# lucian-ilie/SAGE2

Hardware: AMD Instinct MI355X
Metric: overlaps/sec + edge-set bit-identity vs OpenMP ref, 150 bp reads k=40 (higher is better)
Workload: dtype u64

## Files before the change

### sage2_amd/csrc/kernels_index.inc

```


__device__ __forceinline__ void entry_key(const u64* __restrict__ reads, int S, int h, u64 id, int t, u64& hi, u64& lo) {
    const u64* w = reads + id * S;
    int L = (int)(w[S - 1] & slot_len_mask(S));
    u64 phi, plo;
    if (t == 0 || t == 3) key_at(w, S, 0, h, phi, plo); else key_at(w, S, L - h, h, phi, plo);
    if (t >= 2) rc_key(phi, plo, h, hi, lo); else { hi = phi; lo = plo; }
}

__device__ __forceinline__ u64 quad_word(const ulonglong2& v, int q) {
    const u64 a = __shfl(v.x, q >> 1, 4), b = __shfl(v.y, q >> 1, 4);
    return (q & 1) ? b : a;
}
__device__ __forceinline__ void quad_key_at(const ulonglong2& v, int j, int h, u64& hi, u64& lo) {
    const int q = (2 * j) >> 6, r = (2 * j) & 63;
    const u64 w0 = quad_word(v, q);
    u64 w1 = quad_word(v, q + 1 < 8 ? q + 1 : q); w1 = q + 1 < 8 ? w1 : 0ull;
    const u64 a = (w0 << r) | ((w1 >> 1) >> (63 - r));
    if (h <= 32) { hi = 0; lo = a >> (64 - 2 * h); return; }
    u64 w2 = quad_word(v, q + 2 < 8 ? q + 2 : q); w2 = q + 2 < 8 ? w2 : 0ull;
    const u64 b = (w1 << r) | ((w2 >> 1) >> (63 - r));
    const int d = 2 * h - 64;
    hi = a >> (64 - d); lo = d == 64 ? b : ((a << d) | (b >> (64 - d)));
}
// ... 37 lines not shown
__global__ __launch_bounds__(PT_THREADS) void k_ix_tuples(const u64* __restrict__ reads, const u32* __restrict__ posOf, int byPos, u32 N, int S, int h, u64 seed, u32 Th, int wantMI, int shift0, u32 mask0, int doHist,
                                                         u32* T, u32* cnt, u32 ntiles) {
    __shared__ u32 hst[PT_NB_MAX];
    if (doHist) { for (u32 x = threadIdx.x; x <= mask0; x += PT_THREADS) hst[x] = 0; __syncthreads(); }
    if (S == 8) ix_quad_tile<false>(reads, posOf, byPos, N, h, seed, Th, wantMI, shift0, mask0, doHist, T, hst, nullptr);
    else {
#pragma unroll 1
    for (int j = 0; j < PT_TILE / 4 / PT_THREADS; j++) {
        const u32 id0 = blockIdx.x * (PT_TILE / 4) + j * PT_THREADS + threadIdx.x;
        if (id0 >= N) continue;
        const u64 id = (u64)id0 + 1;
        const u64 pos = posOf[id]; const u64 ent4 = pos * 4;
        const u64* w = reads + (byPos ? pos : id) * S;
        const int L = (int)(w[S - 1] & slot_len_mask(S));
        u64 khi[4], klo[4];
        key_at(w, S, 0, h, khi[0], klo[0]); key_at(w, S, L - h, h, khi[1], klo[1]);
        rc_key(khi[1], klo[1], h, khi[2], klo[2]); rc_key(khi[0], klo[0], h, khi[3], klo[3]);
        u32 kk[4], mm[4]; u64 pp[4];
#pragma unroll
        for (int t = 0; t < 4; t++) {
            const u64 hv = hash_key(khi[t], klo[t], h, seed);
            kk[t] = __umulhi((u32)(hv >> 32), Th);
            pp[t] = ((u64)tag_of(hv) << 32) | (u64)(u32)(ent4 + (u64)t);
            mm[t] = 0;
            if (wantMI) { u32 k0, k1, k2, k3; key_left_align(khi[t], klo[t], h, k0, k1, k2, k3); mm[t] = minim_hash(key_min_hash(k0, k1, k2, k3, h), (u32)seed); }
            if (doHist) atomicAdd(&hst[pt_digit(kk[t], shift0, mask0)], 1u);
        }
        if (wantMI) {
#pragma unroll
            for (int t = 0; t < 4; t++) ((uint4*)T)[4 * (u64)id0 + t] = make_uint4(kk[t], mm[t], (u32)pp[t], (u32)(pp[t] >> 32));
        } else {
            u32* o = T + 12 * (u64)id0;
#pragma unroll
            for (int t = 0; t < 4; t++) { o[3 * t] = kk[t]; o[3 * t + 1] = (u32)pp[t]; o[3 * t + 2] = (u32)(pp[t] >> 32); }
        }
    }
    }
    if (doHist) { __syncthreads(); for (u32 x = threadIdx.x; x <= mask0; x += PT_THREADS) cnt[(u64)x * ntiles + blockIdx.x] = hst[x]; }
}
__global__ __launch_bounds__(PT_THREADS) void k_ix_tuples_loc(const u64* __restrict__ reads, const u32* __restrict__ posOf, u32 N, int h, u64 seed, u32 Th, int wantMI, int shift0, u32 mask0, int doHist,
                                                             u32* T, u32* cnt, u32 ntiles, u64* loc) {
    __shared__ u32 hst[PT_NB_MAX];
    if (doHist) { for (u32 x = threadIdx.x; x <= mask0; x += PT_THREADS) hst[x] = 0; __syncthreads(); }
    if (blockIdx.x == 0 && threadIdx.x < 4) ((ulonglong2*)loc)[(u64)posOf[0] * 4 + threadIdx.x] = ((const ulonglong2*)reads)[threadIdx.x];
    ix_quad_tile<true>(reads, posOf, 0, N, h, seed, Th, wantMI, shift0, mask0, doHist, T, hst, loc);
    if (doHist) { __syncthreads(); for (u32 x = threadIdx.x; x <= mask0; x += PT_THREADS) cnt[(u64)x * ntiles + blockIdx.x] = hst[x]; }
}

__global__ void k_debug_table(const u64* __restrict__ slots, u64 T, u64* out) {
    for (u64 idx = (u64)blockIdx.x * blockDim.x + threadIdx.x; idx < T; idx += (u64)gridDim.x * blockDim.x) {
        u64 s = slots[idx]; if (s == 0) continue;
        u32 c7 = (u32)(s >> SLOT_CNT_SHIFT) & 127u;
        atomicAdd(&out[0], 1ull);
        if (c7 == 1) atomicAdd(&out[1], 1ull);
        if (c7 == 0) atomicAdd(&out[2], 1ull);
        if ((s >> SLOT_TAG_SHIFT) == 0) atomicAdd(&out[3], 1ull);
        if (c7 >= 2 && c7 < 127) atomicAdd(&out[4], (u64)c7);
    }
}
__global__ void k_debug_keys(const u64* __restrict__ reads, u64 N, int S, int h, u64* out) {
    u64 e = (u64)blockIdx.x * blockDim.x + threadIdx.x;
    if (e >= 4 * N) return;
    u64 hi, lo; entry_key(reads, S, h, (e >> 2) + 1, (int)(e & 3), hi, lo);
    out[2 * e] = hi; out[2 * e + 1] = lo;
}
template <int NWAVES> __device__ __forceinline__ u32 block_excl_scan(u32 v, u32* sh, u32& total);

constexpr int IXW_CNT_BITS_DEFAULT = 20, IXW_CNT_BITS_WIDE = 30;
__device__ u32 g_fp_mask = 0xFFFFFu;
constexpr int IXW_T = 256;
constexpr int IXW_R = 3072 / IXW_T;
constexpr int IXW_CSR_CAP = 3072;
constexpr u32 GT_INVALID = 0x80000000u;
struct IxWinArgs {
    const u32* T; int W;
    const u32* winOff; u32 nW;
    u64* slots; u32* csr; u64* counters; u64* big; u32 big_cap;
    const u32* idOf;
    u32* G;
    u32 cntBits;
    u64* wh; u64 wh_cap;
};
constexpr int IXW_WAVES = 1;
__global__ __launch_bounds__(IXW_T, IXW_WAVES) void k_ix_window(IxWinArgs A) {
    __shared__ u64 tbl[IX_W];
    __shared__ u32 csrL[IXW_CSR_CAP];
    __shared__ unsigned short csrT[IXW_CSR_CAP];
    __shared__ u32 sh[IXW_T / 64]; __shared__ u64 shWh;
    const u32 tid = threadIdx.x;
    const bool hasM = A.G != nullptr;
    auto tuple = [&](u64 i, u32& k, u64& p, u32& m) {
        if (A.W == 4) { const uint4 v = ((const uint4*)A.T)[i]; k = v.x; m = v.y; p = ((u64)v.w << 32) | v.z; }
        else { const u32* q = A.T + 3 * i; k = q[0]; m = 0; p = ((u64)q[2] << 32) | q[1]; }
    };
    const int IXW_FP_SHIFT = (int)A.cntBits; const u64 IXW_CNT = (1ull << A.cntBits) - 1ull, IXW_FP_MASK = (1ull << (40 - A.cntBits)) - 1ull;
    const u32 fpMask = g_fp_mask & (u32)IXW_FP_MASK;
    u64 accCsr = 0, accOcc = 0;
    for (u32 w = blockIdx.x; w < A.nW; w += gridDim.x) {
        for (u32 x = tid; x < (u32)IX_W; x += IXW_T) tbl[x] = 0ull;
        __syncthreads();
        const u32 b = A.winOff[w], e = A.winOff[w + 1];
        u64 whBase = 0;
        if (e - b > (u32)IXW_R * (u32)IXW_T) {
            if (tid == 0) { const u64 need = (u64)(e - b) - (u64)IXW_R * (u64)IXW_T; u64 at = atomicAdd((unsigned long long*)&A.counters[9], (unsigned long long)need);
                            if (at + need > A.wh_cap) { atomicAdd(&A.counters[8], 1ull << 40); at = ~0ull; } shWh = at; }
            __syncthreads();
            whBase = shWh;
            __syncthreads();
            if (whBase == ~0ull) continue;
        }
        auto insert = [&](u32 k, u64 p, u32 m, u32& info, u32& rank) {
            const u64 tag = p >> 32; const u64 fp = (u64)((m ^ (m >> 20)) & fpMask);
            u32 idx = (k & (u32)(IX_WP - 1)) * 2u; bool files = false; u32 rk = 0; u32 steps = 0;
            for (;;) {
                u64 s = tbl[idx];
                if (s == 0) {
                    s = atomicCAS((unsigned long long*)&tbl[idx], 0ull, (unsigned long long)((tag << SLOT_TAG_SHIFT) | (fp << IXW_FP_SHIFT) | 1ull));
                    if (s == 0) { files = true; break; }
                }
                if ((s >> SLOT_TAG_SHIFT) == tag) {
                    rk = (u32)(atomicAdd((unsigned long long*)&tbl[idx], 1ull) & IXW_CNT);
                    if (rk >= (u32)IXW_CNT - 8u) atomicAdd(&A.counters[8], 1ull << 20);
                    files = ((s >> IXW_FP_SHIFT) & IXW_FP_MASK) != fp;
                    break;
                }
                idx = (idx + 1u) & (u32)(IX_W - 1);
                if (++steps > (u32)IX_W) { atomicAdd(&A.counters[8], 1ull); idx = ~0u; break; }
            }
            info = idx == ~0u ? ~0u : (idx | (files ? 0x80000000u : 0u)); rank = rk;
        };
        u64 cp[IXW_R]; u32 cm[IXW_R], ci[IXW_R], cr[IXW_R]; u32 ck[IXW_R];
#pragma unroll
        for (int r = 0; r < IXW_R; r++) {
            const u32 i = b + (u32)r * (u32)IXW_T + tid; const bool v = i < e;
            ck[r] = 0; cp[r] = 0; cm[r] = 0; if (v) tuple(i, ck[r], cp[r], cm[r]);
        }
#pragma unroll
        for (int r = 0; r < IXW_R; r++) {
            ci[r] = ~0u; cr[r] = 0;
            if (b + (u32)r * (u32)IXW_T + tid < e) insert(ck[r], cp[r], cm[r], ci[r], cr[r]);
        }
        for (u64 i = (u64)b + (u64)IXW_R * (u64)IXW_T + tid; i < e; i += IXW_T) {
            u32 info, rank; u32 tk, tm; u64 tp; tuple(i, tk, tp, tm); insert(tk, tp, tm, info, rank);
            A.wh[whBase + (i - b - (u64)IXW_R * (u64)IXW_T)] = (u64)info | ((u64)rank << 32);
        }
        __syncthreads();
        u32 c[IX_W / IXW_T]; u32 need = 0, occ = 0;
#pragma unroll
        for (int x = 0; x < IX_W / IXW_T; x++) { c[x] = (u32)(tbl[x * IXW_T + tid] & IXW_CNT); need += c[x] >= 2 ? c[x] : 0u; occ += c[x] != 0; }
        u32 total; const u32 excl = block_excl_scan<IXW_T / 64>(need, sh, total);
        u32 occTotal; block_excl_scan<IXW_T / 64>(occ, sh, occTotal);
        accCsr += total; accOcc += occTotal;
        const u64 csrBase = b;
        const bool staged = total <= (u32)IXW_CSR_CAP && (e - b) <= 65535u;
        {
            u64 start = csrBase + excl;
#pragma unroll
            for (int x = 0; x < IX_W / IXW_T; x++) {
                if (c[x] == 0) continue;
                const u32 idx = x * IXW_T + tid; const u64 tagbits = tbl[idx] & (~0ull << SLOT_TAG_SHIFT);
                if (c[x] == 1) tbl[idx] = tagbits | (1ull << SLOT_CNT_SHIFT);
                else {
                    const u32 c7 = c[x] >= HASH_THRESHOLD ? SLOT_CNT_LONG : c[x];
                    tbl[idx] = tagbits | ((u64)c7 << SLOT_CNT_SHIFT) | start;
                    if (c[x] >= HASH_THRESHOLD) {
                        const u64 bb = atomicAdd((unsigned long long*)&A.counters[2], 1ull);
                        if (bb < A.big_cap) { A.big[3 * bb] = (u64)w * IX_W + idx; A.big[3 * bb + 1] = start; A.big[3 * bb + 2] = c[x]; }
                    }
                    start += c[x];
                }
            }
        }
        __syncthreads();
        auto place = [&](u64 i, u64 p, u32 m, u32 info, u32 rank) {
            bool files = false; u64 word = 0;
            if (info != ~0u) {
                const u32 idx = info & 0x7FFFFFFFu; files = (info >> 31) != 0;
                word = tbl[idx]; const u32 c7 = (u32)(word >> SLOT_CNT_SHIFT) & 127u; const u32 entry = (u32)p;
                if (c7 == 1) { word |= (u64)entry; tbl[idx] = word; }
                else { const u64 pos = (word & SLOT_PAY_MASK) + rank; if (staged) { csrL[(u32)(pos - csrBase)] = entry; csrT[(u32)(pos - csrBase)] = (unsigned short)(i - b); } else A.csr[pos] = entry; }
            }
            if (hasM) { u32* g = A.G + 3 * i; g[0] = files ? (m >> 1) : GT_INVALID; g[1] = files ? (u32)word : 0u; g[2] = files ? (u32)(word >> 32) : 0u; }
        };
#pragma unroll
        for (int r = 0; r < IXW_R; r++) { const u64 i = (u64)b + (u64)r * (u64)IXW_T + tid; if (i < e) place(i, cp[r], cm[r], ci[r], cr[r]); }
        for (u64 i = (u64)b + (u64)IXW_R * (u64)IXW_T + tid; i < e; i += IXW_T) { const u64 wv = A.wh[whBase + (i - b - (u64)IXW_R * (u64)IXW_T)]; u32 tk, tm; u64 tp; tuple(i, tk, tp, tm); place(i, tp, tm, (u32)wv, (u32)(wv >> 32)); }
        __syncthreads();
        auto okey = [&](u32 en) -> u64 { return ((u64)A.idOf[en >> 2] << 2) | (u64)(en & 3u); };
#pragma unroll 1
        for (int x = 0; x < IX_W / IXW_T; x++) {
            if (c[x] < 2 || c[x] >= HASH_THRESHOLD) continue;
            const u64 st = tbl[x * IXW_T + tid] & SLOT_PAY_MASK;
            if (staged) {
                u32* a = csrL + (u32)(st - csrBase); unsigned short* ti = csrT + (u32)(st - csrBase);
                for (u32 i = 1; i < c[x]; i++) { const u32 v = a[i]; const unsigned short kv = ti[i]; int j = (int)i - 1; while (j >= 0 && ti[j] > kv) { a[j + 1] = a[j]; ti[j + 1] = ti[j]; j--; } a[j + 1] = v; ti[j + 1] = kv; }
            } else {
                u32* a = A.csr + st;
                for (u32 i = 1; i < c[x]; i++) { const u32 v = a[i]; const u64 kv = okey(v); int j = (int)i - 1; while (j >= 0 && okey(a[j]) > kv) { a[j + 1] = a[j]; j--; } a[j + 1] = v; }
            }
        }
        __syncthreads();
#pragma unroll
        for (int x = 0; x < IX_W / IXW_T; x++) A.slots[(u64)w * IX_W + x * IXW_T + tid] = tbl[x * IXW_T + tid];
        if (staged) for (u32 x = tid; x < total; x += IXW_T) A.csr[csrBase + x] = csrL[x];
        __syncthreads();
    }
    if (tid == 0) { if (accCsr) atomicAdd((unsigned long long*)&A.counters[0], (unsigned long long)accCsr); if (accOcc) atomicAdd((unsigned long long*)&A.counters[1], (unsigned long long)accOcc); }
}

__global__ void k_index_purity(const u64* __restrict__ reads, int S, int h, const u64* __restrict__ big, u64 nbig, const u32* __restrict__ csr, u64* counters) {
    u64 b = ((u64)blockIdx.x * blockDim.x + threadIdx.x) >> 6;
    if (b >= nbig) return;
    u64 start = big[3 * b + 1], c = big[3 * b + 2];
    u32 e0 = csr[start]; u64 hi0, lo0; entry_key(reads, S, h, e0 >> 2, e0 & 3, hi0, lo0);
    bool bad = false;
    for (u64 x = lane_id(); x < c; x += 64) { u32 e = csr[start + x]; u64 hi, lo; entry_key(reads, S, h, e >> 2, e & 3, hi, lo); if (hi != hi0 || lo != lo0) bad = true; }
    if (__ballot(bad)) { if (lane_id() == 0) atomicAdd(&counters[3], 1ull); }
    else if (lane_id() == 0) atomicAdd(&counters[4], 1ull);
}

constexpr u64 BUILD_CNT_MASK = (1ull << SLOT_TAG_SHIFT) - 1;
constexpr int MIW_R = 8;
constexpr int MIW_REC_CAP = 3064;
struct MiWinArgs { const u32* G; const u32* gOff; u32 gW; int tlBits; u64* mi1; u64* krec; u64* counters; u64* wh; u64 wh_cap; };
__global__ __launch_bounds__(256) void k_mi_window(MiWinArgs A) {
    __shared__ u64 tbl[IX_GW];
    __shared__ u64 recL[MIW_REC_CAP];
    __shared__ u32 sh[4]; __shared__ u64 shWh;
    const u32 tid = threadIdx.x; const u32 mtagMask = g_mtag_mask;
    u64 accOcc = 0, accRec = 0;
    for (u32 w = blockIdx.x; w < A.gW; w += gridDim.x) {
        for (u32 x = tid; x < (u32)IX_GW; x += 256) tbl[x] = 0ull;
        __syncthreads();
        const u32 b = A.gOff[w], e = A.gOff[w + 1];
        u64 whBase = 0;
        if (e - b > (u32)MIW_R * 256u) {
            if (tid == 0) { const u64 need = (u64)(e - b) - (u64)MIW_R * 256u; u64 at = atomicAdd((unsigned long long*)&A.counters[9], (unsigned long long)need);
                            if (at + need > A.wh_cap) { atomicAdd(&A.counters[7], 1ull); at = ~0ull; } shWh = at; }
            __syncthreads();
            whBase = shWh;
            __syncthreads();
            if (whBase == ~0ull) continue;
        }
        auto insert = [&](u32 mh1, u32& info, u32& rank) {
            const u64 mt = minim_tag_m(mh1 << 1, mtagMask);
            u32 idx = (mh1 >> (31 - A.tlBits)) & (u32)(IX_GW - 1); u32 rk = 0, steps = 0;
            for (;;) {
                u64 s = tbl[idx];
                if (s == 0) { s = atomicCAS((unsigned long long*)&tbl[idx], 0ull, (unsigned long long)((mt << SLOT_TAG_SHIFT) | 1ull)); if (s == 0) break; }
                if ((s >> SLOT_TAG_SHIFT) == mt) { rk = (u32)(atomicAdd((unsigned long long*)&tbl[idx], 1ull) & BUILD_CNT_MASK); break; }
                idx = (idx + 1u) & (u32)(IX_GW - 1);
                if (++steps > (u32)IX_GW) { atomicAdd(&A.counters[7], 1ull); idx = ~0u; break; }
            }
            info = idx; rank = rk;
        };
        u64 cp[MIW_R]; u32 ck[MIW_R], ci[MIW_R], cr[MIW_R];
#pragma unroll
        for (int r = 0; r < MIW_R; r++) { const u32 i = b + (u32)r * 256u + tid; const bool v = i < e; const u32* g = A.G + 3 * (u64)(v ? i : 0u); ck[r] = v ? g[0] : 0u; cp[r] = v ? (((u64)g[2] << 32) | g[1]) : 0ull; }
#pragma unroll
        for (int r = 0; r < MIW_R; r++) { ci[r] = ~0u; cr[r] = 0; if (b + (u32)r * 256u + tid < e) insert(ck[r], ci[r], cr[r]); }
        for (u64 i = (u64)b + (u64)MIW_R * 256u + tid; i < e; i += 256) { u32 info, rank; insert(A.G[3 * i], info, rank); A.wh[whBase + (i - b - (u64)MIW_R * 256u)] = (u64)info | ((u64)rank << 32); }
        __syncthreads();
        u32 c[IX_GW / 256]; u32 need = 0, occ = 0;
#pragma unroll
        for (int x = 0; x < IX_GW / 256; x++) { const u64 cc = tbl[x * 256 + tid] & BUILD_CNT_MASK; c[x] = cc > 0xFFFFFFFFull ? 0xFFFFFFFFu : (u32)cc; need += c[x]; occ += c[x] != 0; }
        u32 total; const u32 excl = block_excl_scan<4>(need, sh, total);
        u32 occTotal; block_excl_scan<4>(occ, sh, occTotal);
        accOcc += occTotal; accRec += e - b;
        const bool staged = (e - b) <= (u32)MIW_REC_CAP;
        {
            u32 start = b + excl;
#pragma unroll
            for (int x = 0; x < IX_GW / 256; x++) {
                if (c[x] == 0) continue;
                const u32 idx = x * 256 + tid;
                tbl[idx] = (tbl[idx] & (~0ull << SLOT_TAG_SHIFT)) | ((u64)(c[x] >= MI_BIG ? MI_BIG : c[x]) << 32) | (u64)start;
                start += c[x];
            }
        }
        __syncthreads();
        auto place = [&](u64 rec, u32 info, u32 rank) {
            if (info == ~0u) return;
            const u32 pos = (u32)tbl[info] + rank;
            if (staged) recL[pos - b] = rec; else A.krec[pos] = rec;
        };
#pragma unroll
// ... 35 lines not shown
```

### sage2_amd/csrc/sage2ov_device.hip

```cpp
#include <hip/hip_runtime.h>
#include <algorithm>
#include <cstdio>
#include <cstring>
#include <cstdlib>
#include <vector>
#include <chrono>
#include <memory>
#include <atomic>
#include <thread>
#include <sched.h>
#include <pthread.h>
#include <sys/mman.h>
#include "sage2ov.h"
#include "sage2ov_internal.h"

namespace s2 {

#define HIPCHK(call)                                                                                   \
    do {                                                                                               \
        hipError_t e_ = (call);                                                                        \
        if (e_ != hipSuccess) {                                                                        \
            char b_[512];                                                                              \
            snprintf(b_, sizeof b_, "%s:%d %s -> %s", __FILE__, __LINE__, #call, hipGetErrorString(e_)); \
            err = b_;                                                                                  \
// ... 571 lines not shown
static void pt_first_digit(u64 nWin, int shiftW, int* shift0, u32* mask0, int* doHist) {
    int wb, nd; pt_digits(nWin, &wb, &nd);
    if (!nd) { *shift0 = 0; *mask0 = 0; *doHist = 0; return; }
    const int bper = (wb + nd - 1) / nd; *shift0 = shiftW; *mask0 = (1u << std::min(bper, wb)) - 1u; *doHist = 1;
}

static inline double RUN_START_RULE(double f) { return f > 0.1 ? 27.0 * (f - 0.1) : 0.0; }
int dev_build_index(Device* d, uint64_t* slots_out, uint64_t* keys_out, uint64_t* csr_out, uint64_t* nlong_out, uint32_t* rebuilds, std::string& err) {
    HIPCHK(hipSetDevice(d->ordinal));
    const u64 N = d->N; if (!d->reads && !d->readsLoc) { err = "reads not resident"; return SAGE2OV_ERR_ARG; }
    s4cache_release(d);
    HIPCHK(hipEventRecord(d->ev[0], d->stream));
    if (d->diet) {
        HIPCHK(hipStreamSynchronize(d->stream));
        if (!d->resCarved) { hipFree(d->right); hipFree(d->left); hipFree(d->conn); hipFree(d->cflag); hipFree(d->status); hipFree(d->cand);
                             d->right = d->left = nullptr; d->conn = d->cflag = nullptr; d->status = nullptr; d->cand = nullptr; d->cand_cap = 0; d->n_cand = 0; }
        ph_begin(d);
    }
    const u64 fusedThreads = ((4 * N + PT_TILE - 1) / PT_TILE) * PT_THREADS;
    bool copyPending = d->reads && d->S == 8 && !d->diet && N > 0 && fusedThreads < (1ull << 32) && !d->opt.get("SAGE2OV_INDEX_SEPARATE_PASSES");
    if (d->reads) { int rc = build_locality_store(d, copyPending, err); if (rc) return rc; }
    if (d->diet && d->reads && d->uniL) { HIPCHK(hipStreamSynchronize(d->stream)); hipFree(d->reads); d->reads = nullptr; }
    const bool byPos = d->reads == nullptr;
    d->T = std::max<u64>(IX_W, (8 * N + IX_W - 1) / IX_W * IX_W);
    if (const char* ev = d->opt.get("SAGE2OV_TEST_TABLE_SLOTS")) { const u64 want = strtoull(ev, nullptr, 10); if (want > d->T) d->T = (want + IX_W - 1) / IX_W * IX_W; }
    if ((d->T >> 1) >= (1ull << 32)) {
        if (copyPending) hipLaunchKernelGGL(k_loc_scatter, dim3(grid_for_capped((N + 1) * (d->S / 2), 256)), dim3(256), 0, d->stream, d->reads, d->posOf, (u64)N, d->S, d->readsLoc);
        err = "table too large: more than 2^32 slot pairs"; return SAGE2OV_ERR_LIMIT; }
    const u64 nW = d->T / IX_W; const u32 n = (u32)(4 * N);
    const u32 big_cap = 1u << 20;
    WS(slots_ws, u64, WS_SLOTS, d->T); d->slots = slots_ws;
    WS(big, u64, WS_BIG, (u64)big_cap * 3);
    WS(csr_ws, u32, WS_CSR, std::max<u64>(1, 4 * N)); d->csr = csr_ws;
    if (d->runStartsValid) {
        HIPCHK(hipEventSynchronize(d->evRunStarts));
        u64 rs = 0; for (int x = 0; x < 64; x++) rs += d->h_runStarts[x];
        u64 sampled = 0; for (u64 b0 = 0; b0 * 256 < N; b0 += 8) sampled += std::min<u64>(256, N - b0 * 256);
        d->runStartFrac = sampled ? (double)rs / (double)sampled : 0.0; d->runStartsValid = false;
    }
    const double f_ = d->runStartFrac, sizeFactor = N >= 20000000ull ? 1.0 : 0.72;
    bool wantMI = !d->diet && N >= 2000000ull && d->probeShare * sizeFactor * RUN_START_RULE(f_) >= 1.0;
    if (d->opt.get("SAGE2OV_TIMING")) fprintf(stderr, "[index] reads without a predecessor in the locality order: %.1f %% -> minimiser groups %s\n", 100.0 * f_, wantMI ? "built" : "not built");
    if (const char* ev = d->opt.get("SAGE2OV_MINIMIZER_INDEX")) wantMI = atoi(ev) != 0;
    if ((d->h - std::min(d->h, 16) + 1) < 8) wantMI = false;
    u64 TL = 0; int tlBits = 0; u64 gW = 0;
    if (wantMI) { TL = IX_GW; tlBits = IX_GWLOG; while (TL < d->T / 8 * 3) { TL <<= 1; tlBits++; } gW = TL / IX_GW; }
    const u64 nAlloc = std::max<u64>(4, (u64)n + 4);
    const u32 ntiles = (u32)((n + PT_TILE - 1) / PT_TILE);
    PtBufs B; B.W = wantMI ? 4 : 3;
    { WS(a, u32, WS_PT_K0, nAlloc * B.W); B.E[0] = a; } { WS(a, u32, WS_PT_K1, nAlloc * B.W); B.E[1] = a; }
    WS(cnt, u32, WS_PT_CNT, (u64)PT_NB_MAX * std::max<u32>(ntiles, 1) + 2); WS(base, u32, WS_PT_BASE, (u64)PT_NB_MAX * std::max<u32>(ntiles, 1) + 2);
    WS(winOff, u32, WS_PT_OFF, nW + 2);
    u64* mi1 = nullptr; u64* krec = nullptr; u32* gOff = nullptr;
    if (wantMI) {
        WS(m1, u64, WS_MI1, TL); mi1 = m1;
        WS(kr_, u64, WS_KREC, 4 * N + MI_SCAN_PAD); krec = kr_;
        WS(go, u32, WS_PT_GOFF, gW + 3); gOff = go;
    }
    *rebuilds = 0;
    const bool timing = d->opt.get("SAGE2OV_TIMING") != nullptr; auto tp = std::chrono::steady_clock::now();
    auto lap = [&](const char* what) { if (!timing) return; hipStreamSynchronize(d->stream); auto t = std::chrono::steady_clock::now(); fprintf(stderr, "[index] %-34s %8.3f ms\n", what, std::chrono::duration<double, std::milli>(t - tp).count()); tp = t; };
    u64 c[9]; u32 ixCntBits = (u32)IXW_CNT_BITS_DEFAULT;
    for (int attempt = 0;; attempt++) {
        HIPCHK(hipMemsetAsync(d->d_counters + CTR_INDEX, 0, 10 * sizeof(u64), d->stream));
        int shift0, doHist; u32 mask0; pt_first_digit(nW, IX_WPLOG, &shift0, &mask0, &doHist);
        if (copyPending) { hipLaunchKernelGGL(k_ix_tuples_loc, dim3(ntiles), dim3(PT_THREADS), 0, d->stream, d->reads, d->posOf, (u32)N, d->h, d->seed, (u32)(d->T >> 1), wantMI ? 1 : 0, shift0, mask0, doHist,
                                              B.E[0], cnt, ntiles, d->readsLoc); copyPending = false; }
        else if (n) hipLaunchKernelGGL(k_ix_tuples, dim3(ntiles), dim3(PT_THREADS), 0, d->stream, byPos ? d->readsLoc : d->reads, d->posOf, byPos ? 1 : 0, (u32)N, d->S, d->h, d->seed, (u32)(d->T >> 1), wantMI ? 1 : 0, shift0, mask0, doHist,
                                  B.E[0], cnt, ntiles);
        lap("tuples");
        int cur = 0;
        { int rc = partition_by_window(d, B, 0, n, IX_WPLOG, nW, doHist != 0, cnt, base, winOff, &cur, err); if (rc) return rc; }
        lap("partition by table window");
        if (d->opt.get("SAGE2OV_VERIFY_PARTITION") && n) {
            u64* vo = nullptr; HIPCHK(hipMalloc(&vo, 3 * sizeof(u64))); HIPCHK(hipMemsetAsync(vo, 0, 3 * sizeof(u64), d->stream));
            hipLaunchKernelGGL(k_pt_verify, dim3(grid_for(n, 256)), dim3(256), 0, d->stream, B.E[cur], n, IX_WPLOG, (u32)B.W, winOff, (u32)nW, vo);
            u64 hv[3]; HIPCHK(hipMemcpyAsync(hv, vo, sizeof hv, hipMemcpyDeviceToHost, d->stream)); HIPCHK(hipStreamSynchronize(d->stream)); hipFree(vo);
            fprintf(stderr, "[verify-partition] %llu tuples, %llu windows: %llu order violations, largest window %llu tuples, %llu negative windows\n", (unsigned long long)n, (unsigned long long)nW,
                    (unsigned long long)hv[0], (unsigned long long)hv[1], (unsigned long long)hv[2]);
        }
        IxWinArgs A; A.T = B.E[cur]; A.W = B.W; A.winOff = winOff; A.nW = (u32)nW; A.slots = d->slots; A.csr = d->csr;
        A.counters = d->d_counters + CTR_INDEX; A.big = big; A.big_cap = big_cap; A.idOf = d->idOf; A.G = wantMI ? B.E[cur ^ 1] : nullptr; A.wh = nullptr; A.cntBits = ixCntBits;
        { const u64 whCap = n <= (64u << 20) ? nAlloc : nAlloc / 8; WS(whs, u64, WS_WHERE, whCap); A.wh = whs; A.wh_cap = whCap; }
        hipLaunchKernelGGL(k_ix_window, dim3((unsigned)std::min<u64>(nW, 256ull * 6)), dim3(IXW_T), 0, d->stream, A);
        HIPCHK(hipGetLastError());
        HIPCHK(hipMemcpyAsync(c, d->d_counters + CTR_INDEX, sizeof c, hipMemcpyDeviceToHost, d->stream));
        u64 c9 = 0; HIPCHK(hipMemcpyAsync(&c9, d->d_counters + CTR_INDEX + 9, sizeof c9, hipMemcpyDeviceToHost, d->stream));
        HIPCHK(hipStreamSynchronize(d->stream));
        lap("table windows"); mem_sample(d);
        if (c[8] && (c[8] & 0xFFFFFull) == 0 && (c[8] >> 40) == 0 && ixCntBits == (u32)IXW_CNT_BITS_DEFAULT) {
            if (timing) fprintf(stderr, "[index] a key occurs in more than 2^20 reads: building again with the wide counter split\n");
            ixCntBits = (u32)IXW_CNT_BITS_WIDE; attempt--; continue; }
        if (c[8]) { char b_[256]; snprintf(b_, sizeof b_, "index build: %llu table windows overflowed, %llu keys occur in more than 2^30 reads, %llu heavy windows found no scratch (cursor %llu of %llu)",
                             (unsigned long long)(c[8] & 0xFFFFF), (unsigned long long)((c[8] >> 20) & 0xFFFFF), (unsigned long long)(c[8] >> 40), (unsigned long long)c9, (unsigned long long)A.wh_cap);
                    err = b_; return SAGE2OV_ERR_LIMIT; }
        if (c[2] > big_cap) { err = "too many long buckets"; return SAGE2OV_ERR_LIMIT; }
        if (c[2]) {
            hipLaunchKernelGGL(k_index_purity, dim3(grid_for(c[2] * 64, 256)), dim3(256), 0, d->stream, d->readsLoc, d->S, d->h, big, c[2], d->csr, d->d_counters + CTR_INDEX);
            HIPCHK(hipMemcpyAsync(c, d->d_counters + CTR_INDEX, 5 * sizeof(u64), hipMemcpyDeviceToHost, d->stream));
            HIPCHK(hipStreamSynchronize(d->stream));
        }
        if (c[3] == 0) { d->n_csr = c[0]; d->n_keys = c[1]; d->n_long = c[2];
            d->mi1 = nullptr; d->krec = nullptr; d->TL = 0; d->n_groups = 0;
            if (wantMI && d->n_keys > 0) {
                const u32 nG = n;
                PtBufs G; G.W = 3; G.E[0] = B.E[cur ^ 1]; G.E[1] = B.E[cur];
                int gcur = 0; const int gshift = 31 - (tlBits - IX_GWLOG);
                { int rc = partition_by_window(d, G, 0, nG, gshift, gW + 1, false, cnt, base, gOff, &gcur, err); if (rc) return rc; }
                lap("partition by group window");
                MiWinArgs MA; MA.G = G.E[gcur]; MA.gOff = gOff; MA.gW = (u32)gW; MA.tlBits = tlBits; MA.mi1 = mi1; MA.krec = krec; MA.counters = d->d_counters + CTR_INDEX; MA.wh = A.wh; MA.wh_cap = A.wh_cap;
                HIPCHK(hipMemsetAsync(d->d_counters + CTR_INDEX + 9, 0, sizeof(u64), d->stream));
                hipLaunchKernelGGL(k_mi_window, dim3((unsigned)std::min<u64>(gW, 256ull * 8)), dim3(256), 0, d->stream, MA);
                u64 mc[3];
                HIPCHK(hipMemcpyAsync(mc, d->d_counters + CTR_INDEX + 5, sizeof mc, hipMemcpyDeviceToHost, d->stream));
                HIPCHK(hipStreamSynchronize(d->stream));
                HIPCHK(hipMemsetAsync(krec + mc[0], 0, MI_SCAN_PAD * sizeof(u64), d->stream));
                lap("group windows"); mem_sample(d);
                d->n_groups = mc[1];
                if (d->opt.get("SAGE2OV_VERIFY_MI")) {
                    u64* vo = nullptr; HIPCHK(hipMalloc(&vo, 2 * sizeof(u64))); HIPCHK(hipMemsetAsync(vo, 0, 2 * sizeof(u64), d->stream));
                    hipLaunchKernelGGL(k_mi_verify, dim3(grid_for(4 * N, 256)), dim3(256), 0, d->stream, d->readsLoc, N, d->S, d->h, d->seed, d->slots, d->T, mi1, TL, krec, vo);
                    u64 hv2[2]; HIPCHK(hipMemcpyAsync(hv2, vo, sizeof hv2, hipMemcpyDeviceToHost, d->stream)); HIPCHK(hipStreamSynchronize(d->stream)); hipFree(vo);
                    fprintf(stderr, "[verify-mi] %llu of %llu entries do not find their bucket in their key's group\n", (unsigned long long)hv2[0], (unsigned long long)hv2[1]);
                }
                if (mc[2] == 0 && mc[1] * 10 <= TL * 7) { d->mi1 = mi1; d->krec = krec; d->TL = TL; }
                if (timing) fprintf(stderr, "[index] minimiser groups: %llu groups, %llu records, %llu group words (load %.2f), crowded windows %llu -> %s\n", (unsigned long long)mc[1], (unsigned long long)mc[0],
                                    (unsigned long long)TL, (double)mc[1] / (double)TL, (unsigned long long)mc[2], d->mi1 ? "used" : "NOT used");
            }
            break;
        }
        if (attempt >= 8) { err = "index build: tag collisions in long buckets persist after 8 reseeds"; return SAGE2OV_ERR_INTERNAL; }
        d->seed = d->seed * 0x9E3779B97F4A7C15ull + 12345; (*rebuilds)++;
    }
    HIPCHK(hipEventRecord(d->ev[1], d->stream));
    HIPCHK(hipStreamSynchronize(d->stream));
    float ms = 0; hipEventElapsedTime(&ms, d->ev[0], d->ev[1]); d->tm.index_ms += ms;
    if (d->diet) ph_begin(d);
    *slots_out = d->T; *keys_out = d->n_keys; *csr_out = d->n_csr; *nlong_out = d->n_long;
    return 0;
}

int dev_lookup(Device* d, uint64_t hi, uint64_t lo, uint64_t* entries, uint32_t cap, uint32_t* count, std::string& err) {
    HIPCHK(hipSetDevice(d->ordinal));
    if (!d->slots) { err = "index not built"; return SAGE2OV_ERR_ARG; }
    u64* out = nullptr; const u32 c2 = std::min<u32>(cap, 128);
    HIPCHK(hipMalloc(&out, (129) * sizeof(u64)));
    hipLaunchKernelGGL(k_lookup, dim3(1), dim3(1), 0, d->stream, d->slots, d->T, d->csr, d->idOf, d->seed, d->h, (u64)hi, (u64)lo, out, c2);
    u64 host[129];
    HIPCHK(hipMemcpyAsync(host, out, sizeof host, hipMemcpyDeviceToHost, d->stream));
    HIPCHK(hipStreamSynchronize(d->stream));
    hipFree(out);
    *count = (u32)host[0];
    for (u32 x = 0; x < *count && x < c2; x++) entries[x] = host[1 + x];
    return 0;
}

template <int MODE>
static int launch_probe(Device* d, ProbeArgs& A, std::string& err) {
    const u64 nreads = A.ids ? A.n_ids : A.hi - A.lo; if (nreads == 0) return 0;
    const unsigned wpb = d->S == 32 ? 1 : (d->S == 16 ? 2 : 4);
    const unsigned blocks = (unsigned)std::min<u64>((nreads + wpb - 1) / wpb, 256ull * 32);
    switch (d->S) {
        case 4: hipLaunchKernelGGL((k_probe<4, MODE, 4>), dim3(blocks), dim3(256), 0, d->stream, A); break;
        case 8: hipLaunchKernelGGL((k_probe<8, MODE, 4>), dim3(blocks), dim3(256), 0, d->stream, A); break;
        case 16: hipLaunchKernelGGL((k_probe<16, MODE, 2>), dim3(blocks), dim3(128), 0, d->stream, A); break;
        case 32: hipLaunchKernelGGL((k_probe<32, MODE, 1>), dim3(blocks), dim3(64), 0, d->stream, A); break;
        default: err = "bad S"; return SAGE2OV_ERR_INTERNAL;
    }
    HIPCHK(hipGetLastError());
    return 0;
}
static ProbeArgs base_args(Device* d) {
// ... 2579 lines not shown
```

Baseline: 62.25 billion.

## Template window index kernel with prefetched tuples and batched LDS hash inserts

Turns the window-table build kernel into a template with serial, plain and grouped forms, picked at launch by the default path. The new forms prefetch the next window's bounds and tuples before the table clear, and issue all register-resident inserts as concurrent LDS CAS rounds with a single waitcnt per round instead of a serial probe loop per tuple. They also raise the occupancy hint in launch bounds, specialise the tuple width at compile time, and pass the slot word into place separately. The cost is more code paths and heavier register use, plus reliance on inline asm and waitcnt encodings.

```diff
diff --git a/sage2_amd/csrc/kernels_index.inc b/sage2_amd/csrc/kernels_index.inc
--- a/sage2_amd/csrc/kernels_index.inc
+++ b/sage2_amd/csrc/kernels_index.inc
@@ -143,24 +143,48 @@
     u64* wh; u64 wh_cap;
 };
 constexpr int IXW_WAVES = 1;
-__global__ __launch_bounds__(IXW_T, IXW_WAVES) void k_ix_window(IxWinArgs A) {
+constexpr int IXW_SERIAL = 0, IXW_PLAIN = 1, IXW_GROUPS = 2;
+constexpr int IXW_WAVES_ROUNDS = 3;
+constexpr int IXW_WAIT_LDS = 0xC07F;
+template <int FORM>
+__global__ __launch_bounds__(IXW_T, FORM == IXW_SERIAL ? IXW_WAVES : FORM == IXW_GROUPS ? 2 : IXW_WAVES_ROUNDS) void k_ix_window(IxWinArgs A) {
+    constexpr bool ROUNDS = FORM != IXW_SERIAL, GROUPS = FORM == IXW_GROUPS;
     __shared__ u64 tbl[IX_W];
     __shared__ u32 csrL[IXW_CSR_CAP];
     __shared__ unsigned short csrT[IXW_CSR_CAP];
     __shared__ u32 sh[IXW_T / 64]; __shared__ u64 shWh;
     const u32 tid = threadIdx.x;
-    const bool hasM = A.G != nullptr;
+    const bool hasM = ROUNDS ? GROUPS : A.G != nullptr;
     auto tuple = [&](u64 i, u32& k, u64& p, u32& m) {
-        if (A.W == 4) { const uint4 v = ((const uint4*)A.T)[i]; k = v.x; m = v.y; p = ((u64)v.w << 32) | v.z; }
+        if (ROUNDS ? GROUPS : A.W == 4) { const uint4 v = ((const uint4*)A.T)[i]; k = v.x; m = v.y; p = ((u64)v.w << 32) | v.z; }
         else { const u32* q = A.T + 3 * i; k = q[0]; m = 0; p = ((u64)q[2] << 32) | q[1]; }
     };
     const int IXW_FP_SHIFT = (int)A.cntBits; const u64 IXW_CNT = (1ull << A.cntBits) - 1ull, IXW_FP_MASK = (1ull << (40 - A.cntBits)) - 1ull;
     const u32 fpMask = g_fp_mask & (u32)IXW_FP_MASK;
     u64 accCsr = 0, accOcc = 0;
+    u64 cp[IXW_R]; u32 cm[IXW_R], ci[IXW_R], cr[IXW_R]; u32 ck[IXW_R];
+    u32 ce[IXW_R], ct[IXW_R];
+    u32 nb = 0, ne = 0;
+    auto next_bounds = [&](u32 wn) { nb = 0; ne = 0; if (wn < A.nW) { nb = A.winOff[wn]; ne = A.winOff[wn + 1]; } };
+    auto opaque_tid = [&]() -> u32 { u32 t = tid; asm volatile("" : "+v"(t)); return t; };
+    auto load_tuples = [&]() {
+        constexpr int W = GROUPS ? 4 : 3;
+        const u32 t = opaque_tid();
+        const u32* w0 = A.T + (u64)W * nb; const u32* mine = w0 + W * t;
+        const int nreg = (int)min(ne - nb, (u32)IXW_R * (u32)IXW_T);
+#pragma unroll
+        for (int r = 0; r < IXW_R; r++) {
+            const u32* q = (int)t < nreg - r * IXW_T ? mine + W * r * IXW_T : w0;
+            if (GROUPS) { const uint4 v = *(const uint4*)q; ck[r] = v.x; cm[r] = v.y; ce[r] = v.z; ct[r] = v.w; }
+            else { ck[r] = q[0]; cm[r] = 0; ce[r] = q[1]; ct[r] = q[2]; }
+        }
+    };
+    if (ROUNDS) next_bounds(blockIdx.x);
     for (u32 w = blockIdx.x; w < A.nW; w += gridDim.x) {
+        if (ROUNDS) load_tuples();
         for (u32 x = tid; x < (u32)IX_W; x += IXW_T) tbl[x] = 0ull;
         __syncthreads();
-        const u32 b = A.winOff[w], e = A.winOff[w + 1];
+        const u32 b = ROUNDS ? nb : A.winOff[w], e = ROUNDS ? ne : A.winOff[w + 1];
         u64 whBase = 0;
         if (e - b > (u32)IXW_R * (u32)IXW_T) {
             if (tid == 0) { const u64 need = (u64)(e - b) - (u64)IXW_R * (u64)IXW_T; u64 at = atomicAdd((unsigned long long*)&A.counters[9], (unsigned long long)need);
@@ -168,7 +192,7 @@
             __syncthreads();
             whBase = shWh;
             __syncthreads();
-            if (whBase == ~0ull) continue;
+            if (whBase == ~0ull) { if (ROUNDS) next_bounds(w + gridDim.x); continue; }
         }
         auto insert = [&](u32 k, u64 p, u32 m, u32& info, u32& rank) {
             const u64 tag = p >> 32; const u64 fp = (u64)((m ^ (m >> 20)) & fpMask);
@@ -190,21 +214,63 @@
             }
             info = idx == ~0u ? ~0u : (idx | (files ? 0x80000000u : 0u)); rank = rk;
         };
-        u64 cp[IXW_R]; u32 cm[IXW_R], ci[IXW_R], cr[IXW_R]; u32 ck[IXW_R];
-#pragma unroll
-        for (int r = 0; r < IXW_R; r++) {
-            const u32 i = b + (u32)r * (u32)IXW_T + tid; const bool v = i < e;
-            ck[r] = 0; cp[r] = 0; cm[r] = 0; if (v) tuple(i, ck[r], cp[r], cm[r]);
-        }
-#pragma unroll
-        for (int r = 0; r < IXW_R; r++) {
-            ci[r] = ~0u; cr[r] = 0;
-            if (b + (u32)r * (u32)IXW_T + tid < e) insert(ck[r], cp[r], cm[r], ci[r], cr[r]);
+        if (!ROUNDS) {
+#pragma unroll
+            for (int r = 0; r < IXW_R; r++) {
+                const u32 i = b + (u32)r * (u32)IXW_T + tid; const bool v = i < e;
+                ck[r] = 0; cp[r] = 0; cm[r] = 0; if (v) tuple(i, ck[r], cp[r], cm[r]);
+            }
+#pragma unroll
+            for (int r = 0; r < IXW_R; r++) {
+                ci[r] = ~0u; cr[r] = 0;
+                if (b + (u32)r * (u32)IXW_T + tid < e) insert(ck[r], cp[r], cm[r], ci[r], cr[r]);
+            }
+        } else {
+            u32 pend = 0, steps = 0; const u32 t = opaque_tid(); const int nreg = (int)min(e - b, (u32)IXW_R * (u32)IXW_T);
+            u32 cwh[IXW_R], joined = 0; u64 s[IXW_R];
+            auto fp_of = [&](int r) -> u64 { return GROUPS ? (u64)((cm[r] ^ (cm[r] >> 20)) & fpMask) : 0ull; };
+            auto word = [&](int r) -> u64 { return ((u64)cwh[r] << 32) | (u64)((u32)(fp_of(r) << IXW_FP_SHIFT) | 1u); };
+            auto is_empty = [&](u64 v) -> bool { u32 lo = (u32)v; asm volatile("" : "+v"(lo)); return lo == 0; };
+            auto same_tag = [&](u64 v, int r) -> bool { return (((u32)(v >> 32) ^ cwh[r]) >> (SLOT_TAG_SHIFT - 32)) == 0; };
+            auto other_key = [&](u64 v, int r) -> bool { return GROUPS && ((u32)(v >> IXW_FP_SHIFT) & (u32)IXW_FP_MASK) != (u32)fp_of(r); };
+#pragma unroll
+            for (int r = 0; r < IXW_R; r++) {
+                cwh[r] = (ct[r] << (SLOT_TAG_SHIFT - 32)) | (u32)((fp_of(r) << IXW_FP_SHIFT) >> 32);
+                ci[r] = (ck[r] & (u32)(IX_WP - 1)) * 2u; s[r] = 0; if ((int)t < nreg - r * IXW_T) pend |= 1u << r;
+            }
+#pragma unroll
+            for (int r = 0; r < IXW_R; r++) if ((pend >> r) & 1u) s[r] = atomicCAS((unsigned long long*)&tbl[ci[r]], 0ull, (unsigned long long)word(r));
+            while (pend && steps <= (u32)IX_W) {
+                __builtin_amdgcn_s_waitcnt(IXW_WAIT_LDS);
+#pragma unroll
+                for (int r = 0; r < IXW_R; r++) if ((pend >> r) & 1u) {
+                    const u64 v = s[r];
+                    if (is_empty(v)) { ci[r] |= 0x80000000u; pend &= ~(1u << r); }
+                    else if (same_tag(v, r)) {
+                        if (other_key(v, r)) ci[r] |= 0x80000000u;
+                        cwh[r] = atomicAdd((u32*)&tbl[ci[r] & 0x7FFFFFFFu], 1u); joined |= 1u << r;
+                        pend &= ~(1u << r);
+                    }
+                    else { ci[r] = (ci[r] + 1u) & (u32)(IX_W - 1); s[r] = atomicCAS((unsigned long long*)&tbl[ci[r]], 0ull, (unsigned long long)word(r)); }
+                }
+                steps++;
+            }
+            __builtin_amdgcn_s_waitcnt(IXW_WAIT_LDS);
+            if (pend) {
+#pragma unroll
+                for (int r = 0; r < IXW_R; r++) if ((pend >> r) & 1u) { atomicAdd(&A.counters[8], 1ull); ci[r] = ~0u; }
+            }
+#pragma unroll
+            for (int r = 0; r < IXW_R; r++) {
+                cr[r] = ((joined >> r) & 1u) ? cwh[r] & (u32)IXW_CNT : 0u;
+                if (cr[r] >= (u32)IXW_CNT - 8u) atomicAdd(&A.counters[8], 1ull << 20);
+            }
         }
         for (u64 i = (u64)b + (u64)IXW_R * (u64)IXW_T + tid; i < e; i += IXW_T) {
             u32 info, rank; u32 tk, tm; u64 tp; tuple(i, tk, tp, tm); insert(tk, tp, tm, info, rank);
             A.wh[whBase + (i - b - (u64)IXW_R * (u64)IXW_T)] = (u64)info | ((u64)rank << 32);
         }
+        if (ROUNDS) next_bounds(w + gridDim.x);
         __syncthreads();
         u32 c[IX_W / IXW_T]; u32 need = 0, occ = 0;
 #pragma unroll
@@ -226,26 +292,37 @@
                     tbl[idx] = tagbits | ((u64)c7 << SLOT_CNT_SHIFT) | start;
                     if (c[x] >= HASH_THRESHOLD) {
                         const u64 bb = atomicAdd((unsigned long long*)&A.counters[2], 1ull);
-                        if (bb < A.big_cap) { A.big[3 * bb] = (u64)w * IX_W + idx; A.big[3 * bb + 1] = start; A.big[3 * bb + 2] = c[x]; }
+                        if (bb < A.big_cap) { A.big[3 * bb] = ((u64)w * IX_W + tid) + (u64)(x * IXW_T); A.big[3 * bb + 1] = start; A.big[3 * bb + 2] = c[x]; }
                     }
                     start += c[x];
                 }
             }
         }
         __syncthreads();
-        auto place = [&](u64 i, u64 p, u32 m, u32 info, u32 rank) {
-            bool files = false; u64 word = 0;
-            if (info != ~0u) {
+        auto place = [&](u64 i, u64 p, u32 m, u32 info, u32 rank, u64 word) {
+            bool files = false;
+            if (info == ~0u) word = 0;
+            else {
                 const u32 idx = info & 0x7FFFFFFFu; files = (info >> 31) != 0;
-                word = tbl[idx]; const u32 c7 = (u32)(word >> SLOT_CNT_SHIFT) & 127u; const u32 entry = (u32)p;
+                const u32 c7 = (u32)(word >> SLOT_CNT_SHIFT) & 127u; const u32 entry = (u32)p;
                 if (c7 == 1) { word |= (u64)entry; tbl[idx] = word; }
                 else { const u64 pos = (word & SLOT_PAY_MASK) + rank; if (staged) { csrL[(u32)(pos - csrBase)] = entry; csrT[(u32)(pos - csrBase)] = (unsigned short)(i - b); } else A.csr[pos] = entry; }
             }
             if (hasM) { u32* g = A.G + 3 * i; g[0] = files ? (m >> 1) : GT_INVALID; g[1] = files ? (u32)word : 0u; g[2] = files ? (u32)(word >> 32) : 0u; }
         };
-#pragma unroll
-        for (int r = 0; r < IXW_R; r++) { const u64 i = (u64)b + (u64)r * (u64)IXW_T + tid; if (i < e) place(i, cp[r], cm[r], ci[r], cr[r]); }
-        for (u64 i = (u64)b + (u64)IXW_R * (u64)IXW_T + tid; i < e; i += IXW_T) { const u64 wv = A.wh[whBase + (i - b - (u64)IXW_R * (u64)IXW_T)]; u32 tk, tm; u64 tp; tuple(i, tk, tp, tm); place(i, tp, tm, (u32)wv, (u32)(wv >> 32)); }
+        auto slot_word = [&](u32 info) -> u64 { return info != ~0u ? tbl[info & 0x7FFFFFFFu] : 0ull; };
+        if (!ROUNDS) {
+#pragma unroll
+            for (int r = 0; r < IXW_R; r++) { const u64 i = (u64)b + (u64)r * (u64)IXW_T + tid; if (i < e) place(i, cp[r], cm[r], ci[r], cr[r], slot_word(ci[r])); }
+        } else {
+            u64 wd[IXW_R]; const int nreg = (int)min(e - b, (u32)IXW_R * (u32)IXW_T);
+            const u32 t = opaque_tid(), i0 = b + t;
+#pragma unroll
+            for (int r = 0; r < IXW_R; r++) { wd[r] = 0; if ((int)t < nreg - r * IXW_T) wd[r] = slot_word(ci[r]); }
+#pragma unroll
+            for (int r = 0; r < IXW_R; r++) if ((int)t < nreg - r * IXW_T) place((u64)(i0 + (u32)(r * IXW_T)), (u64)ce[r], cm[r], ci[r], cr[r], wd[r]);
+        }
+        for (u64 i = (u64)b + (u64)IXW_R * (u64)IXW_T + tid; i < e; i += IXW_T) { const u64 wv = A.wh[whBase + (i - b - (u64)IXW_R * (u64)IXW_T)]; u32 tk, tm; u64 tp; tuple(i, tk, tp, tm); place(i, tp, tm, (u32)wv, (u32)(wv >> 32), slot_word((u32)wv)); }
         __syncthreads();
         auto okey = [&](u32 en) -> u64 { return ((u64)A.idOf[en >> 2] << 2) | (u64)(en & 3u); };
 #pragma unroll 1
@@ -262,7 +339,7 @@
         }
         __syncthreads();
 #pragma unroll
-        for (int x = 0; x < IX_W / IXW_T; x++) A.slots[(u64)w * IX_W + x * IXW_T + tid] = tbl[x * IXW_T + tid];
+        for (int x = 0; x < IX_W / IXW_T; x++) (A.slots + ((u64)w * IX_W + tid))[x * IXW_T] = tbl[x * IXW_T + tid];
         if (staged) for (u32 x = tid; x < total; x += IXW_T) A.csr[csrBase + x] = csrL[x];
         __syncthreads();
     }
diff --git a/sage2_amd/csrc/sage2ov_device.hip b/sage2_amd/csrc/sage2ov_device.hip
--- a/sage2_amd/csrc/sage2ov_device.hip
+++ b/sage2_amd/csrc/sage2ov_device.hip
@@ -677,12 +677,16 @@
         IxWinArgs A; A.T = B.E[cur]; A.W = B.W; A.winOff = winOff; A.nW = (u32)nW; A.slots = d->slots; A.csr = d->csr;
         A.counters = d->d_counters + CTR_INDEX; A.big = big; A.big_cap = big_cap; A.idOf = d->idOf; A.G = wantMI ? B.E[cur ^ 1] : nullptr; A.wh = nullptr; A.cntBits = ixCntBits;
         { const u64 whCap = n <= (64u << 20) ? nAlloc : nAlloc / 8; WS(whs, u64, WS_WHERE, whCap); A.wh = whs; A.wh_cap = whCap; }
-        hipLaunchKernelGGL(k_ix_window, dim3((unsigned)std::min<u64>(nW, 256ull * 6)), dim3(IXW_T), 0, d->stream, A);
+        { const dim3 g((unsigned)std::min<u64>(nW, 256ull * 6));
+          if (d->opt.get("SAGE2OV_IX_WINDOW_SERIAL")) hipLaunchKernelGGL(k_ix_window<IXW_SERIAL>, g, dim3(IXW_T), 0, d->stream, A);
+          else if (wantMI) hipLaunchKernelGGL(k_ix_window<IXW_GROUPS>, g, dim3(IXW_T), 0, d->stream, A);
+          else hipLaunchKernelGGL(k_ix_window<IXW_PLAIN>, g, dim3(IXW_T), 0, d->stream, A); }
         HIPCHK(hipGetLastError());
         HIPCHK(hipMemcpyAsync(c, d->d_counters + CTR_INDEX, sizeof c, hipMemcpyDeviceToHost, d->stream));
         u64 c9 = 0; HIPCHK(hipMemcpyAsync(&c9, d->d_counters + CTR_INDEX + 9, sizeof c9, hipMemcpyDeviceToHost, d->stream));
         HIPCHK(hipStreamSynchronize(d->stream));
         lap("table windows"); mem_sample(d);
+        if (timing) fprintf(stderr, "[index] heavy windows: %llu scratch words drawn\n", (unsigned long long)c9);
         if (c[8] && (c[8] & 0xFFFFFull) == 0 && (c[8] >> 40) == 0 && ixCntBits == (u32)IXW_CNT_BITS_DEFAULT) {
             if (timing) fprintf(stderr, "[index] a key occurs in more than 2^20 reads: building again with the wide counter split\n");
             ixCntBits = (u32)IXW_CNT_BITS_WIDE; attempt--; continue; }
```

Result: no change. 62.69 billion, median of 6 (+0.7%).
